# GiulioRomualdi/paper_romualdi_2022_icra_centroidal-mpc-walking

Hardware: AMD Instinct MI355X
Metric: centroidal-MPC solves/sec (batch, horizon=20) (higher is better)
Workload: dtype f32

## Files before the change

include/cmpc.h:

```cpp
#ifndef CMPC_H
#define CMPC_H

#include <stddef.h>

#ifdef __cplusplus
extern "C" {
#endif

typedef struct cmpc_handle_s* cmpc_handle;

typedef enum {
    CMPC_OK = 0,
    CMPC_ERR_ARG = -1,
    CMPC_ERR_HIP = -2,
    CMPC_ERR_NOT_CONVERGED = -3
} cmpc_status;

typedef struct {
    int horizon;
    double sampling_time;
    double friction_coefficient;
    double gravity;
    double com_weight[3];
    double angular_momentum_weight;
// ... 18 lines not shown
#define CMPC_FACTORS_HBM 2

#define CMPC_INFO 8

void cmpc_default_config(cmpc_config* cfg);
int cmpc_dims(int horizon, int* n_x, int* n_p, int* n_g, int* nnz_jac, int* nnz_hess);

double cmpc_default_tolerance(int horizon);
int cmpc_create(const cmpc_config* cfg, int batch, int device, cmpc_handle* out);
int cmpc_destroy(cmpc_handle h);
const char* cmpc_last_error(cmpc_handle h);
int cmpc_batch(cmpc_handle h);
void* cmpc_stream(cmpc_handle h);

int cmpc_solve_device(cmpc_handle h, const float* dP, const float* dX0, float* dX, float* dInfo,
                      void* stream);
int cmpc_solve_device_warm(cmpc_handle h, const float* dP, const float* dX0, float* dX, float* dInfo,
                           void* stream);
int cmpc_set_warm_policy(cmpc_handle h, int warm_budget, int restart_in_kernel);
int cmpc_solve(cmpc_handle h, const float* P, const float* X0, float* X, float* info);
float cmpc_last_solve_ms(cmpc_handle h);
int cmpc_set_timing(cmpc_handle h, int enabled);
int cmpc_test_poison_lds(cmpc_handle h);

typedef struct {
    double friction_coefficient;
    double com_weight[3];
    double angular_momentum_weight;
    double contact_position_weight;
    double force_rate_of_change_weight[3];
    double contact_force_symmetry_weight;
    double corners[2][4][3];
} cmpc_model;
#define CMPC_MODEL_DOUBLES 34
void cmpc_model_from_config(const cmpc_config* cfg, cmpc_model* model);
int cmpc_check_models(const cmpc_model* models, int batch);
int cmpc_set_models(cmpc_handle h, const cmpc_model* models);
int cmpc_set_models_device(cmpc_handle h, const cmpc_model* dModels, int* dOk, void* stream);

int cmpc_eval_nlp_device(cmpc_handle h, const float* dX, const float* dP, const float* dLamG,
                         float lam_f, float* dF, float* dG, float* dGradF, float* dJac,
                         float* dHess, void* stream);
int cmpc_nlp_sparsity(int horizon, int* jac_row, int* jac_col, int* hess_row, int* hess_col);
int cmpc_eval_nlp_grad_device(cmpc_handle h, const float* dX, const float* dP, const float* dLamG, float lam_f,
                              float* dGradX, float* dGradP, void* stream);

// ... 197 lines not shown
```

paper_romualdi_2022_icra_centroidal-mpc-walking_amd/_capi.py:

```python
from __future__ import annotations

import ctypes as C
import os

_HERE = os.path.dirname(os.path.abspath(__file__))
LIB_PATH = os.path.join(_HERE, os.environ.get("CMPC_LIB", "libcmpc_hip.so"))

INFO = 8
CERT = 8
SENS = 8


class CmpcConfig(C.Structure):
    _fields_ = [
        ("horizon", C.c_int),
        ("sampling_time", C.c_double),
        ("friction_coefficient", C.c_double),
        ("gravity", C.c_double),
        ("com_weight", C.c_double * 3),
        ("angular_momentum_weight", C.c_double),
        ("contact_position_weight", C.c_double),
        ("force_rate_of_change_weight", C.c_double * 3),
        ("contact_force_symmetry_weight", C.c_double),
        ("corners", C.c_double * 24),
# ... 52 lines not shown
class CmpcModel(C.Structure):
    _fields_ = [
        ("friction_coefficient", C.c_double),
        ("com_weight", C.c_double * 3),
        ("angular_momentum_weight", C.c_double),
        ("contact_position_weight", C.c_double),
        ("force_rate_of_change_weight", C.c_double * 3),
        ("contact_force_symmetry_weight", C.c_double),
        ("corners", C.c_double * 24),
    ]


MODEL_DOUBLES = 34


FACTORS = {None: 0, "auto": 0, "lds": 1, "hbm": 2}


EXPORTS = [
    "cmpc_default_config", "cmpc_dims", "cmpc_create", "cmpc_destroy", "cmpc_last_error",
    "cmpc_batch", "cmpc_stream", "cmpc_solve_device", "cmpc_solve", "cmpc_last_solve_ms", "cmpc_set_timing",
    "cmpc_eval_nlp_device", "cmpc_nlp_sparsity", "cmpc_set_state", "cmpc_set_reference",
    "cmpc_set_contacts", "cmpc_set_initial_guess", "cmpc_advance", "cmpc_get_solution",
    "cmpc_get_output", "cmpc_set_reference_from_planner", "cmpc_plant_step_device", "cmpc_test_poison_lds",
    "cmpc_compact_output_device", "cmpc_contacts_merge", "cmpc_contacts_merge_device", "cmpc_contacts_sample",
    "cmpc_contacts_sample_device", "cmpc_set_contact_lists", "cmpc_contacts_adjust", "cmpc_contacts_adjust_device",
    "cmpc_write_state_device", "cmpc_shift_solution_device", "cmpc_eval_nlp_grad_device", "cmpc_solve_device_warm", "cmpc_set_warm_policy",
    "cmpc_get_parameters", "cmpc_get_parameters_device", "cmpc_allgather_compact_device",
    "cmpc_rollout_tick_device", "cmpc_write_reference_from_planner_device", "cmpc_default_tolerance",
    "cmpc_contacts_force_sample_time", "cmpc_contacts_force_sample_time_device",
    "cmpc_model_from_config", "cmpc_check_models", "cmpc_set_models", "cmpc_set_models_device",
    "cmpc_set_multiplier_output", "cmpc_get_multipliers_device", "cmpc_get_multipliers", "cmpc_kkt_certificate_device",
    "cmpc_value_gradient_device", "cmpc_solution_jvp_device", "cmpc_solution_vjp_device",
    "cmpc_sensitivity_workspace_bytes", "cmpc_solution_jvp_model_device", "cmpc_solution_vjp_model_device", "cmpc_model_value_gradient_device",
    "cmpc_plant_step_jvp_device", "cmpc_plant_step_vjp_device", "cmpc_contacts_position_vjp_device", "cmpc_rollout_tick_vjp_device",
    "cmpc_solution_jvp_rot_device", "cmpc_solution_vjp_rot_device", "cmpc_rotation_value_gradient_device", "cmpc_contacts_rotation_vjp_device",
    "cmpc_plant_step_jvp_rot_device", "cmpc_plant_step_vjp_rot_device", "cmpc_contacts_orientation_vjp_device", "cmpc_rollout_tick_vjp_rot_device",
    "cmpc_plant_step_jvp_cols_device", "cmpc_contacts_jvp_device", "cmpc_rollout_tick_jvp_device",
    "cmpc_rollout_record", "cmpc_rollout_record_device", "cmpc_rollout_outcome_init_device", "cmpc_cold_start_device", "cmpc_rollout_walk_device",
]

_lib = None


def lib():
    global _lib
    if _lib is None:
# ... 114 lines not shown
```

paper_romualdi_2022_icra_centroidal-mpc-walking_amd/csrc/cmpc_api.hip:

```cpp
#include "../../include/cmpc.h"
#include "cmpc_contacts.h"
#include "cmpc_device.h"

#include <algorithm>
#include <cmath>
#include <cstdio>
#include <cstdlib>
#include <cstring>
#include <dlfcn.h>
#include <string>
#include <vector>

extern "C" size_t cmpc_solver_lds_bytes(int N, int factors_global);
extern "C" int cmpc_launch_solver(const CmpcParams* prm, size_t lds_bytes, hipStream_t stream);
extern "C" int cmpc_prepare_solver(int N, int factors_global, size_t lds_bytes);
extern "C" int cmpc_launch_nlp_eval(const CmpcParams* prm, const float* dX, const float* dP, const float* dLamG,
                                    float lam_f, float* dF, float* dG, float* dGradF, float* dJac, float* dHess,
                                    hipStream_t stream);
extern "C" int cmpc_launch_nlp_grad(const CmpcParams* prm, const float* dX, const float* dP, const float* dLamG, float lam_f, float* dGradX,
                                    float* dGradP, hipStream_t stream);
extern "C" int cmpc_launch_multipliers(const CmpcParams* prm, const float* dX, const float* dP, float* dLamG, hipStream_t stream);
extern "C" int cmpc_launch_kkt_certificate(const CmpcParams* prm, const float* dX, const float* dP, const float* dLamG, float* dCert, hipStream_t stream);
extern "C" int cmpc_launch_value_gradient(const CmpcParams* prm, const float* dX, const float* dP, const float* dLamG, float* dGradP, hipStream_t stream);
extern "C" int cmpc_launch_sensitivity(const CmpcConsts* kc, int kc_per_problem, int N, int b0, int nb, const float* dX, const float* dP, const float* dLamG,
// ... 673 lines not shown
    int rc = cmpc_launch_nlp_grad(&p, dX, dP, dLamG, lam_f, dGradX, dGradP, stream ? (hipStream_t)stream : h->stream);
    if (rc != 0) return fail(h, CMPC_ERR_HIP, std::string("nlp grad launch: ") + hipGetErrorString((hipError_t)rc));
    return CMPC_OK;
}

int cmpc_set_multiplier_output(cmpc_handle h, int enabled)
{
    if (!h) return fail(h, CMPC_ERR_ARG, "cmpc_set_multiplier_output: null handle");
    HIPCHK(h, hipSetDevice(h->device));
    if (enabled && !h->dDuals) {
        const size_t nd = (size_t)h->B * (CMPC_NS * (h->cfg.horizon + 1) + 2 * CMPC_NI * h->cfg.horizon);
        HIPCHK(h, hipMalloc(&h->dDuals, sizeof(float) * nd));
        HIPCHK(h, hipMemsetAsync(h->dDuals, 0, sizeof(float) * nd, h->stream));
        HIPCHK(h, hipStreamSynchronize(h->stream));
    } else if (!enabled && h->dDuals && !h->warm_duals) {
        HIPCHK(h, hipDeviceSynchronize());
        HIPCHK(h, hipFree(h->dDuals));
        h->dDuals = nullptr;
    }
    h->mult_out = enabled != 0;
    return CMPC_OK;
}

int cmpc_get_multipliers_device(cmpc_handle h, const float* dX, const float* dP, float* dLamG, void* stream)
{
    if (!h || !dX || !dP || !dLamG) return fail(h, CMPC_ERR_ARG, "cmpc_get_multipliers_device: null argument");
    if (!h->mult_out || !h->dDuals) return fail(h, CMPC_ERR_ARG, "cmpc_get_multipliers_device: the multiplier output is off (cmpc_set_multiplier_output)");
    HIPCHK(h, hipSetDevice(h->device));
    CmpcParams p;
    fill_params(h, p);
    int rc = cmpc_launch_multipliers(&p, dX, dP, dLamG, stream ? (hipStream_t)stream : h->stream);
    if (rc != 0) return fail(h, CMPC_ERR_HIP, std::string("multipliers launch: ") + hipGetErrorString((hipError_t)rc));
    return CMPC_OK;
}

int cmpc_get_multipliers(cmpc_handle h, float* LamG)
{
    if (!h || !LamG) return fail(h, CMPC_ERR_ARG, "cmpc_get_multipliers: null argument");
    if (!h->have_solution) return fail(h, CMPC_ERR_ARG, "cmpc_get_multipliers: no solution yet (cmpc_advance)");
    HIPCHK(h, hipSetDevice(h->device));
    const size_t n = (size_t)h->B * h->L.ng;
    if (!h->dLamG) HIPCHK(h, hipMalloc(&h->dLamG, sizeof(float) * n));
    int rc = cmpc_get_multipliers_device(h, h->dX, h->dP, h->dLamG, nullptr);
    if (rc != CMPC_OK) return rc;
    HIPCHK(h, hipMemcpyAsync(LamG, h->dLamG, sizeof(float) * n, hipMemcpyDeviceToHost, h->stream));
    HIPCHK(h, hipStreamSynchronize(h->stream));
// ... 1027 lines not shown
```

paper_romualdi_2022_icra_centroidal-mpc-walking_amd/csrc/cmpc_solver.hip:

```cpp
#include "cmpc_device.h"

#include <cstdlib>
#include <type_traits>
#include <map>
#include <mutex>

#define NS CMPC_NS
#define NF CMPC_NF
#define NQ CMPC_NQ
#define NU CMPC_NU
#define NXA CMPC_NXA
#define NI CMPC_NI
#define PLD 39
#define GLD 30
#define RLD 36
#define NPAN 46
#define GEO 36
#define SQ_TILE_WAVES 6
#define SQ_SPIN_MAX (1 << 20)
#define SQ_PUB_FLOATS (10 * NPAN * 4 + 128 * 4)
#define ZLD 36
#define MSET (NU * RLD + NPAN * RLD + NS * 16)
#define NTRI 256
#define ID_STRIP_LEN 68
#define ID_STRIPS (4 * ID_STRIP_LEN)
#define DSET_F (3 * NU + 3 * NS + 3 + 108)
#define DSET_I (3 * NU + 3 * NS + 3)
#define REC_UB 0
#define REC_WT 576
#define REC_ZERO 572
#define REC_N CMPC_REC_N
constexpr int SWEEP_UNROLL = 4;
constexpr int DELTA_UNROLL = 4;

namespace {

#ifdef CMPC_PROFILE
__device__ long long g_prof[128];
__device__ float g_trace[64 * 8];
#define PROF_DECL long long pt_ = __builtin_amdgcn_s_memtime()
#define PROF(slot) do { long long n_ = __builtin_amdgcn_s_memtime(); if (threadIdx.x == 0 && blockIdx.x == 0) g_prof[slot] += n_ - pt_; pt_ = n_; } while (0)
#define PROF2_DECL long long pt2_ = __builtin_amdgcn_s_memtime()
#define PROF3(slot) do { long long n_ = __builtin_amdgcn_s_memtime(); if (threadIdx.x == 192 && blockIdx.x == 0) g_prof[slot] += n_ - pt2_; pt2_ = n_; } while (0)
#define PROF4(slot) do { long long n_ = __builtin_amdgcn_s_memtime(); if (threadIdx.x == 128 && blockIdx.x == 0) g_prof[slot] += n_ - pt2_; pt2_ = n_; } while (0)
#define PROF2(slot) do { long long n_ = __builtin_amdgcn_s_memtime(); if (threadIdx.x == 0 && blockIdx.x == 0) g_prof[slot] += n_ - pt2_; pt2_ = n_; } while (0)
#define PROF5(slot) do { long long n_ = __builtin_amdgcn_s_memtime(); if (threadIdx.x == 216 && blockIdx.x == 0) g_prof[slot] += n_ - pt2_; pt2_ = n_; } while (0)
#define CPROF(i) do { if (ln == 0 && blockIdx.x == 0 && k < N) atomicAdd(reinterpret_cast<unsigned long long*>(&g_prof[32 + 5 * wv + (i)]), (unsigned long long)(__builtin_amdgcn_s_memtime() - pc0_)); } while (0)
#define CPROF2(i) do { if (ln == 0 && blockIdx.x == 0 && k < N) atomicAdd(reinterpret_cast<unsigned long long*>(&g_prof[64 + 8 * wv + (i)]), (unsigned long long)(__builtin_amdgcn_s_memtime() - pc0_)); } while (0)
#ifdef CMPC_PROFILE_LIGHT
#undef PROF2_DECL
#undef PROF2
#undef PROF3
#undef PROF4
#undef PROF5
#undef CPROF
#undef CPROF2
#define CPROF2(i)
#define PROF2_DECL
#define PROF2(slot)
#define PROF3(slot)
#define PROF4(slot)
#define PROF5(slot)
#define CPROF(i)
#define SQPROF_DECL
#define SQPROF(slot)
#else
#define SQPROF_DECL PROF_DECL
#define SQPROF(slot) PROF(slot)
#endif
#else
#define SQPROF_DECL
#define SQPROF(slot)
#define CPROF(i)
#define CPROF2(i)
#define PROF_DECL
#define PROF(slot)
#define PROF2_DECL
#define PROF2(slot)
#define PROF3(slot)
#define PROF4(slot)
#define PROF5(slot)
#endif

struct Ctx {
    CmpcIdx L;
    int N;
    const float* sp;
    float *S, *U, *T, *Z;
    float* LAM;
    float *dS, *dU, *dT, *dZ, *d;
    float *Lf;
    float *geoA;
    float *P0, *Qb, *G, *QuuF, *Pan, *Bval, *Aval, *arow, *ybuf, *fpv, *fpn;
    float *idstrip;
    float *ZT;
    double *QuuD1, *qs1;
    int *Brow, *Arow, *qmask;
    unsigned short* tri;
    double *QuuD, *pv, *pn, *qs, *Pd, *sig, *gco, *redd;
// ... 133 lines not shown
{
    const auto r = __builtin_amdgcn_permlane32_swap(__float_as_uint(v), __float_as_uint(v), false, false);
    return __uint_as_float(r[0]) + __uint_as_float(r[1]);
}
__device__ inline float oct_sum(float v)
{
    v += __uint_as_float(__builtin_amdgcn_update_dpp(0u, __float_as_uint(v), 0xB1, 0xF, 0xF, true));
    v += __uint_as_float(__builtin_amdgcn_update_dpp(0u, __float_as_uint(v), 0x4E, 0xF, 0xF, true));
    v += __uint_as_float(__builtin_amdgcn_update_dpp(0u, __float_as_uint(v), 0x141, 0xF, 0xF, true));
    return v;
}
__device__ inline float dot4(const float4& a, const float4& b) { return a.x * b.x + a.y * b.y + a.z * b.z + a.w * b.w; }

__device__ inline float gam_of(const Ctx& c, int ct, int k) { return c.sp[c.L.pGam(ct) + k]; }
__device__ inline float Rm(const float* R, int r, int cc) { return R[3 * cc + r]; }

__device__ inline bool qfree_compute(const Ctx& c, int k, int m)
{
    const int ct = m / 3, i = m % 3;
    const float lo = c.sp[c.L.pLo(ct) + 3 * k + i], hi = c.sp[c.L.pUp(ct) + 3 * k + i];
    return gam_of(c, ct, k) < 0.5f && (hi - lo) > 1e-9f;
}
__device__ inline bool qfree(const Ctx& c, int k, int m) { return (c.qmask[k] >> m) & 1; }
__device__ inline bool outside_subset(const Ctx& c, int ct, int k)
{
    const float g = gam_of(c, ct, k);
    if (g == 0.f) return false;
    if (g != 1.f) return true;
    int kp = -1;
    for (int j = k - 1; j >= 0 && kp < 0; --j) if (gam_of(c, ct, j) < 0.5f) kp = j;
    const float* R = c.sp + c.L.pR(ct) + 9 * k;
    const float* nom = c.sp + c.L.pNom(ct) + 3 * (k + 1);
    const float* lo = c.sp + c.L.pLo(ct) + 3 * k;
    const float* up = c.sp + c.L.pUp(ct) + 3 * k;
    if (kp < 0) {
        const float* cur = c.sp + c.L.pCur(ct);
        bool out = false;
        for (int i = 0; i < 3; ++i) {
            float v = 0.f;
            for (int a = 0; a < 3; ++a) v += Rm(R, a, i) * (cur[a] - nom[a]);
            out = out || !(v >= lo[i] - 1e-6f && v <= up[i] + 1e-6f);
        }
        return out;
    }
    const float* Rp = c.sp + c.L.pR(ct) + 9 * kp;
    const float* nomp = c.sp + c.L.pNom(ct) + 3 * (kp + 1);
    const float* lop = c.sp + c.L.pLo(ct) + 3 * kp;
    const float* upp = c.sp + c.L.pUp(ct) + 3 * kp;
    bool diff = false;
    for (int a = 0; a < 9; ++a) diff = diff || __float_as_int(R[a]) != __float_as_int(Rp[a]);
    for (int i = 0; i < 3; ++i)
        diff = diff || __float_as_int(nom[i]) != __float_as_int(nomp[i]) || __float_as_int(lo[i]) != __float_as_int(lop[i])
               || __float_as_int(up[i]) != __float_as_int(upp[i]);
    return diff;
}
__device__ inline float qlo(const Ctx& c, int k, int m) { return c.sp[c.L.pLo(m / 3) + 3 * k + m % 3]; }
__device__ inline float qhi(const Ctx& c, int k, int m) { return c.sp[c.L.pUp(m / 3) + 3 * k + m % 3]; }

__device__ inline void fric_row(const Ctx& c, const CmpcConsts& prm, int k, int i, float& a0, float& a1, float& a2)
{
    const int ct = i >> 4, face = i & 3;
    const float* R = c.sp + c.L.pR(ct) + 9 * k;
    const float sx = (face == 0 || face == 3) ? 1.f : -1.f;
    const float sy = (face < 2) ? 1.f : -1.f;
    const float nmu = -prm.mu_fr;
    a0 = __builtin_fmaf(nmu, Rm(R, 0, 2), __builtin_fmaf(sy, Rm(R, 0, 1), sx * Rm(R, 0, 0)));
    a1 = __builtin_fmaf(nmu, Rm(R, 1, 2), __builtin_fmaf(sy, Rm(R, 1, 1), sx * Rm(R, 1, 0)));
    a2 = __builtin_fmaf(nmu, Rm(R, 2, 2), __builtin_fmaf(sy, Rm(R, 2, 1), sx * Rm(R, 2, 0)));
}

__device__ inline bool row_active(const Ctx& c, int k, int i) { return i < 32 ? true : qfree(c, k, (i - 32) % 6); }

__device__ inline float row_val(const Ctx& c, const CmpcConsts& prm, int k, int i, const float* u)
{
    if (i < 32) {
        float a0, a1, a2;
// ... 2066 lines not shown
{
    CMPC_PHASE_PROLOGUE;
    const bool affine = __builtin_amdgcn_readfirstlane((int)affine_in) != 0;
    riccati_forward<NT, NC == 0 ? 1 : (FG ? 2 : SWEEP_UNROLL), FG, PART>(c, prm, tid, affine, 0);
}
template <int NT, int NC, bool FG>
__device__ __forceinline__ void phase_forward_sweep(lds_t lds, int Nrt, float* fg_base, bool affine_in)
{
    if (threadIdx.x < 64) phase_forward_part<NT, NC, FG, 1>(lds, Nrt, fg_base, affine_in);
}
template <int NT, int NC, bool FG>
__device__ __attribute__((noinline)) void phase_forward_tail(lds_t lds, int Nrt, float* fg_base, bool affine_in, int k0_in)
{
    CMPC_PHASE_PROLOGUE;
    const bool affine = __builtin_amdgcn_readfirstlane((int)affine_in) != 0;
    const int k0 = __builtin_amdgcn_readfirstlane(k0_in);
    riccati_forward<NT, 1, FG>(c, prm, tid, affine, k0);
}
template <int NT, int NC, bool FG>
__device__ __attribute__((noinline)) void phase_delta_part(lds_t lds, int Nrt, float* fg_base)
{
    CMPC_PHASE_PROLOGUE;
    riccati_delta<NC == 0 ? 1 : (FG ? 2 : DELTA_UNROLL), FG>(c, prm, tid);
}
template <int NT, int NC, bool FG>
__device__ __forceinline__ void phase_delta(lds_t lds, int Nrt, float* fg_base)
{
    if (threadIdx.x < 64) phase_delta_part<NT, NC, FG>(lds, Nrt, fg_base);
    __syncthreads();
}
template <int NT, int NC, bool FG>
__device__ __attribute__((noinline)) void phase_costate(lds_t lds, int Nrt, float* fg_base, float ap, bool exact_in)
{
    CMPC_PHASE_PROLOGUE;
    const bool use_exact = __builtin_amdgcn_readfirstlane((int)exact_in) != 0;
    costate_update(c, prm, tid, ap, use_exact);
}
__device__ inline float dual_extrapolate(float z, float dz) { return fmaxf(z + dz, 0.f); }

template <int NT, int NC, bool FG>
__device__ __attribute__((noinline)) void tail_polish(lds_t lds, int Nrt, float* fg_base, int k0_in, bool duals_in)
{
    CMPC_PHASE_PROLOGUE;
    const int k0 = __builtin_amdgcn_readfirstlane(k0_in);
    const bool duals = __builtin_amdgcn_readfirstlane((int)duals_in) != 0;
    bool last = false, blocked = true;
    for (int pi = 0; pi <= prm.tail_iters + 6 && !last; ++pi) {
        last = pi >= prm.tail_iters + 6 || (pi >= prm.tail_iters && !blocked);
        all_geo<NT>(c, prm, tid);
        for (int e = tid + NS * k0; e < NS * N; e += NT) c.d[e] = (float)defect(c, prm, e / NS, e % NS);
        __syncthreads();
// ... 150 lines not shown
        if (e % NU < NF) {
            l_fm = fmaxf(l_fm, fabsf(c.U[e]));
            if (e >= NU * kt) l_tail = fmaxf(l_tail, fabsf(du));
        }
    }
    float m3[3] = {l_all, l_tail, l_fm};
    block_maxn<NT, 3>(m3, c.red, tid);
    if (!(m3[0] < INFINITY)) return false;
    const int k0 = (prm.tail_stages > 0 && m3[1] > prm.tail_trigger * m3[2]) ? kt : N;
    if (k0 < N) step_lengths<NT>(c, tid, 0.999f, ap, ad, 0, k0);
    for (int e = tid; e < NS * (k0 < N ? k0 + 1 : N + 1); e += NT) c.S[e] += ap * c.dS[e];
    for (int e = tid; e < NU * k0; e += NT) c.U[e] += ap * c.dU[e];
    if (duals)
        for (int e = tid; e < NI * k0; e += NT) {
            const float tn = c.T[e] + ap * c.dT[e], zn = dual_extrapolate(c.Z[e], c.dZ[e]);
            if (fabsf(tn) < INFINITY && fabsf(zn) < INFINITY) { c.T[e] = tn; c.Z[e] = zn; }
        }
    __syncthreads();
    if (k0 == N) return false;
    tail_polish<NT, NC, FG>(lds, N, fg_base, k0, duals);
    return true;
}

template <int NT, int NC, bool FG>
__device__ __attribute__((noinline)) int phase_setup(lds_t lds, int Nrt, float* fg_base, const float* gp)
{
    CMPC_PHASE_PROLOGUE;
    float* spw = const_cast<float*>(c.sp);
    for (int e = tid; e < NTRI; e += NT) {
        int i = (int)((sqrtf(8.f * (float)e + 1.f) - 1.f) * 0.5f);
        while ((i + 1) * (i + 2) / 2 <= e) ++i;
        while (i * (i + 1) / 2 > e) --i;
        c.tri[e] = (unsigned short)((i << 8) | (e - i * (i + 1) / 2));
    }
    for (int e = tid; e < ID_STRIPS; e += NT) c.idstrip[e] = (e % ID_STRIP_LEN) == 32 + e / ID_STRIP_LEN ? 1.f : 0.f;
    for (int e = tid; e < c.L.np(); e += NT) spw[e] = gp[e];
    if (tid == 0) c.flag[0] = 0;
    __syncthreads();
    if (tid < N) {
        int m = 0;
#pragma unroll
        for (int q = 0; q < NQ; ++q) m |= qfree_compute(c, tid, q) ? (1 << q) : 0;
        c.qmask[tid] = m;
    }
    if (tid < 2 * N && outside_subset(c, tid / N, tid % N)) c.flag[0] = 1;
    __syncthreads();
    return __builtin_amdgcn_readfirstlane(c.flag[0]);
}

template <int NT, int NC, bool FG>
__device__ __attribute__((noinline)) int phase_init(lds_t lds, int Nrt, float* fg_base, const float* x0, const float* dprev, int flags, float mu_init,
                                                    float t_floor)
{
    CMPC_PHASE_PROLOGUE;
    const bool cold = (flags & 1) != 0, use_duals = (flags & 2) != 0, use_mult = (flags & 4) != 0;
    for (int e = tid; e < NS * (N + 1); e += NT) {
        const int k = e / NS, i = e % NS;
        float v;
        if (k == 0) {
            if (i < 9) v = c.sp[c.L.pCom0() + i];
            else v = c.sp[c.L.pCur((i - 9) / 3) + (i - 9) % 3];
        } else if (cold) v = i < 3 ? c.sp[c.L.pCom0() + i] : (i < 9 ? 0.f : c.sp[c.L.pNom((i - 9) / 3) + 3 * k + (i - 9) % 3]);
        else if (i < 9) v = x0[c.L.oCom() + 3 * (N + 1) * (i / 3) + 3 * k + i % 3];
        else v = x0[c.L.oPos((i - 9) / 3) + 3 * k + (i - 9) % 3];
        c.S[e] = v;
        c.LAM[e] = (use_duals && !cold) ? dprev[NS * (k < N ? k + 1 : N) + i] : 0.f;
    }
    for (int e = tid; e < NU * N; e += NT) {
        const int k = e / NU, m = e % NU;
        float v = 0.f;
        if (m < NF) v = cold ? (m % 3 == 2 ? 0.125f * prm.grav : 0.f) : x0[c.L.oF(m / 12, (m % 12) / 3) + 3 * k + m % 3];
        else {
            const int q = m - 24, ct = q / 3, i = q % 3;
            if (qfree(c, k, q)) {
                const float* R = c.sp + c.L.pR(ct) + 9 * k;
                const float lo = qlo(c, k, q), hi = qhi(c, k, q), push = 0.01f * (hi - lo);
                for (int a = 0; a < 3 && !cold; ++a)
                    v += Rm(R, a, i) * (x0[c.L.oPos(ct) + 3 * (k + 1) + a] - c.sp[c.L.pNom(ct) + 3 * (k + 1) + a]);
                v = fminf(fmaxf(v, lo + push), hi - push);
            } else if (gam_of(c, ct, k) < 0.5f) v = qlo(c, k, q);
        }
        c.U[e] = v;
    }
    __syncthreads();
    for (int e = tid; e < NI * N; e += NT) {
        const int k = e / NI, i = e % NI;
        float t = 1.f, z = 0.f;
        if (row_active(c, k, i)) {
            t = -row_val(c, prm, k, i, c.U + NU * k);
            if (i < 32) t = fmaxf(t, t_floor);
            z = mu_init / t;
            if (use_mult && !cold) {
                const int kk = k + 1 < N ? k + 1 : N - 1;
                z = fmaxf(z, dprev[NS * (N + 1) + NI * N + NI * kk + i]);
            }
        }
        c.T[e] = t; c.Z[e] = z;
    }
    __syncthreads();
    int nrow = 0;
    for (int k = 0; k < N; ++k)
        for (int i = 32; i < NI; ++i) nrow += row_active(c, k, i) ? 1 : 0;
    return __builtin_amdgcn_readfirstlane(nrow + 32 * N);
}

template <int NT, int NC, bool FG>
__device__ __attribute__((noinline)) float phase_multipliers(lds_t lds, int Nrt, float* fg_base, int mode_in, float a_in, int nrow_in)
{
    CMPC_PHASE_PROLOGUE;
    const int mode = __builtin_amdgcn_readfirstlane(mode_in), nrow = __builtin_amdgcn_readfirstlane(nrow_in);
    const float a = uniform_f(a_in);
    float out = a;
    if (mode == 0) {
        for (int e = tid; e < NI * N; e += NT) c.Z[e] *= a;
    } else if (mode == 1) {
        double l2 = 0.0;
        for (int e = tid; e < NI * N; e += NT)
            if (row_active(c, e / NI, e % NI)) {
                const float t = c.T[e];
                float z = c.Z[e];
                if (t * z > 10.f * a) { z = 10.f * a / t; c.Z[e] = z; }
                l2 += (double)t * z;
            }
        out = (float)(block_sum<NT>(l2, c.redd, tid) / (double)nrow);
    } else {
        for (int e = tid; e < NI * N; e += NT) c.dZ[e] = row_active(c, e / NI, e % NI) ? a : 0.f;
// ... 200 lines not shown
            for (int e = tid; e < NS * N; e += NT) c.d[e] = 0.f;
            __syncthreads();
            if (tid < 64) costate_scan<true>(c, prm, tid, 0.f, false, c.LAM);
            __syncthreads();
        }
        for (int e = tid; e < NS * (N + 1); e += NT) dq[e] = e < NS ? (e == 0 ? (float)status : 0.f) : c.LAM[e];
        for (int e = tid; e < NI * N; e += NT) { dq[NS * (N + 1) + e] = c.T[e]; dq[NS * (N + 1) + NI * N + e] = c.Z[e]; }
    }
#ifdef CMPC_PROFILE
    if (prm.hwid_probe) {
        __syncthreads();
        if ((threadIdx.x & 63) == 0) x[threadIdx.x >> 6] = (float)(__builtin_amdgcn_s_getreg((31 << 11) | 4) & 0xffff);
    }
#endif
}

template <int NT, int NC, bool FG>
__global__ __launch_bounds__(NT, FG ? 3 : 1) void cmpc_solve_kernel(CmpcParams kp)
{
    extern __shared__ __attribute__((aligned(16))) char smem[];
    const int b = blockIdx.x;
    const int tid = threadIdx.x;
    const int N = NC > 0 ? NC : kp.N;
    {
        int* z = reinterpret_cast<int*>(smem);
        for (int e = tid; e < kp.lds_words; e += NT) z[e] = 0;
    }
    __syncthreads();
    {
        const int* src = reinterpret_cast<const int*>(kp.kc_per_problem ? kp.kc + b : kp.kc);
        int* dst = reinterpret_cast<int*>(smem);
        for (int e = tid; e < (int)(sizeof(CmpcConsts) / 4); e += NT) dst[e] = src[e];
    }
    const CmpcConsts& prm = *reinterpret_cast<const CmpcConsts*>(smem);
    const long long t_start = __builtin_amdgcn_s_memtime();
    unsigned ldsv = (unsigned)(unsigned long long)(lds_t)smem;
    asm volatile("" : "+s"(ldsv));
    const lds_t lds = (lds_t)(unsigned long long)ldsv;
    float* const fg_base = FG ? kp.scratch + (size_t)b * kp.scratch_stride : nullptr;
    const CmpcIdx L{N};
    __syncthreads();
    const bool outside = (phase_setup<NT, NC, FG>(lds, N, fg_base, kp.P + (size_t)b * L.np()) != 0) | (prm.model_bad != 0);
    int status = 1, sg = 0, it_total = 0;
    float err = 0.f, ep = 0.f, mu_cur = 0.f, step_out = 0.f, step_prev = 0.f;
    float* const dq = kp.duals ? kp.duals + (size_t)b * (NS * (N + 1) + 2 * NI * N) : nullptr;
    if (outside) {
        phase_init<NT, NC, FG>(lds, N, fg_base, kp.X0 + (size_t)b * L.nx(), dq, 0, kp.mu_init, kp.t_floor);
        status = 3;
    }
    for (int pass = 0; pass < 2 && !outside; ++pass) {
        const float mu_init = pass ? 0.1f : kp.mu_init, t_floor = pass ? 1e-2f : kp.t_floor, mu_adapt = pass ? 3.5f : kp.mu_adapt;
        step_out = step_prev = 0.f;
        const bool use_duals = kp.warm && kp.warm_duals && kp.duals;
        const int nrow = phase_init<NT, NC, FG>(lds, N, fg_base, kp.X0 + (size_t)b * L.nx(), dq,
                                                (pass > 0 ? 1 : 0) | (use_duals ? 2 : 0) | (use_duals && kp.warm_duals > 1 ? 4 : 0), mu_init, t_floor);
        int it = 0;
        status = 1;
        bool finishing = false;
        const int budget = (kp.warm && pass == 0 && kp.warm_budget > 0 && kp.warm_budget < prm.max_iter) ? kp.warm_budget : prm.max_iter;
        for (it = 0; it < budget + 1; ++it) {
            if (it == budget && !finishing) break;
            PROF_DECL;
            const Resid rs = phase_residuals<NT, NC, FG>(lds, N, fg_base, nrow);
            ep = rs.ep;
            const float ec = rs.ec;
            mu_cur = rs.mu;
            if (!(ep < INFINITY)) { status = 2; err = INFINITY; break; }
            if (it == 0 && mu_adapt > 0.f) {
                const float mu0 = fminf(fmaxf(mu_adapt * ep * ep, 0.03f), 0.5f);
                phase_multipliers<NT, NC, FG>(lds, N, fg_base, 0, mu0 / mu_cur, nrow);
                mu_cur = mu0;
            }
            if (kp.warm && pass == 0 && it > 0 && ec > 100.f * mu_cur && ec > 0.1f) {
                mu_cur = phase_multipliers<NT, NC, FG>(lds, N, fg_base, 1, mu_cur, nrow);
                sg += 100;
            }
            PROF(10);
            float est = step_out;
// ... 13 lines not shown
            int fail = 1;
            bool resync = false;
            for (int attempt = 0; attempt < 4; ++attempt) {
                fail = phase_backward<NT, NC, FG>(lds, N, fg_base, exact, reg, centring ? prm.mu_min : 0.f);
                if (!fail) break;
                __syncthreads();
                if (fail & 2) {
                    sg += 1000000;
                    if (!resync) { resync = true; --attempt; continue; }
                }
                ++sg; exact = false;
                if (attempt > 0) reg *= 1e3f;
            }
            if (fail) { if (!finishing) status = 2; break; }
            PROF(11);
            float sigma = 0.f, mu_t = prm.mu_min;
            if (centring) {
                phase_multipliers<NT, NC, FG>(lds, N, fg_base, 2, prm.mu_min, nrow);
            } else {
                phase_forward_sweep<NT, NC, FG>(lds, N, fg_base, true);
                PROF(12);
                if (finishing) {
                    phase_forward_part<NT, NC, FG, 2>(lds, N, fg_base, true);
                    if (phase_finish<NT, NC, FG>(lds, N, fg_base, dq != nullptr)) sg += 100000;
                    ++it;
                    break;
                }
                Centre ce;
                if constexpr (NC > 0) ce = phase_affine_post<NT, NC, FG>(lds, N, fg_base, mu_cur, nrow);
                else {
                    phase_forward_part<NT, NC, FG, 2>(lds, N, fg_base, true);
                    const StepLen sa = phase_step_lengths<NT, NC, FG>(lds, N, fg_base, 1.f);
                    ce = phase_corrector_targets<NT, NC, FG>(lds, N, fg_base, sa.ap, sa.ad, mu_cur, nrow);
                }
                sigma = ce.sigma; mu_t = ce.mu_t;
                PROF(13);
                phase_delta<NT, NC, FG>(lds, N, fg_base);
                PROF(14);
            }
            phase_forward_sweep<NT, NC, FG>(lds, N, fg_base, false);
            PROF(15);
            float ap, ad, step;
            if constexpr (NC > 0) {
                const FinalStep fs = phase_final_post<NT, NC, FG>(lds, N, fg_base, fmaxf(0.99f, 1.f - mu_t), exact);
                ap = fs.ap; ad = fs.ad; step = fs.step;
                PROF(16);
            } else {
// ... 5 lines not shown
                step = phase_update<NT, NC, FG>(lds, N, fg_base, ap, ad);
            }
            step_prev = step_out;
            step_out = step;
            err = fmaxf(ep, ec);
    #ifdef CMPC_PROFILE
            if (tid == 0 && b == 0 && it < 64) {
                float* tr = g_trace + 8 * it;
                tr[0] = mu_cur; tr[1] = ep; tr[2] = ec; tr[3] = step; tr[4] = ap; tr[5] = ad; tr[6] = sigma; tr[7] = mu_t;
            }
    #endif
            PROF(17);
            if (err <= prm.tol && step <= prm.step_tol) {
                status = 0;
                if (!prm.final_extrap) { ++it; break; }
                finishing = true;
            }
        }
        it_total += it;
        if (status == 0 || !kp.warm || pass > 0 || kp.warm_no_restart) break;
        sg += 10000;
        __syncthreads();
    }
    phase_export<NT, NC, FG>(lds, N, fg_base, kp.X + (size_t)b * L.nx(), dq, status);
    if (kp.info && tid == 0) {
        float* inf = kp.info + (size_t)b * CMPC_INFO_N;
        inf[0] = (float)it_total; inf[1] = err; inf[2] = mu_cur; inf[3] = (float)sg; inf[4] = ep; inf[5] = (float)status;
        inf[6] = (float)(__builtin_amdgcn_s_memtime() - t_start); inf[7] = step_out;
    }
}

}

extern "C" size_t cmpc_solver_lds_bytes(int N, int factors_global)
{
    CmpcLayout L;
    cmpc_layout_init(L, N);
    const size_t dbl = 90 + 40 + 40 + 16 + 40 + 4 * NI + 8 + (factors_global ? 0 : 90 + 16);
    const size_t work = factors_global ? ((NXA * PLD + 3) & ~3) + NS * 16 + ((NXA * GLD + 3) & ~3) : (size_t)MSET + NS * 16 + SQ_PUB_FLOATS + 128;
    const size_t flt = (size_t)NU * RLD + (size_t)NPAN * RLD + 96 + ID_STRIPS + ((L.np + 3) & ~3)
                       + ((size_t)NS * (N + 1) + (size_t)NU * N + ((factors_global && N > CMPC_TZ_LDS_NMAX) ? 0 : 2 * (size_t)NI * N)) + (size_t)NS * N + (size_t)NS * (N + 1)
                       + (size_t)GEO * N + work + 2 * DSET_F + 40 + 40 + 24
                       + 2 * DSET_I + 4 + CMPC_NMAX + NTRI / 2 + (factors_global ? 0 : (size_t)REC_N * N);
    return ((sizeof(CmpcConsts) + 15) & ~(size_t)15) + dbl * 8 + flt * 4;
}

#ifdef CMPC_PROFILE
extern "C" int cmpc_profile_read(long long* out, int reset)
{
    hipError_t e = hipMemcpyFromSymbol(out, HIP_SYMBOL(g_prof), sizeof(long long) * 128);
    if (reset) { long long z[128] = {0}; (void)hipMemcpyToSymbol(HIP_SYMBOL(g_prof), z, sizeof(z)); }
    return (int)e;
}
extern "C" int cmpc_trace_read(float* out) { return (int)hipMemcpyFromSymbol(out, HIP_SYMBOL(g_trace), sizeof(float) * 64 * 8); }
#endif

typedef void (*cmpc_kernel_t)(CmpcParams);
static cmpc_kernel_t solver_variant(int N, bool factors_global, int& nthreads)
{
    constexpr int NT = 256, NR = 512;
    if (factors_global) {
        nthreads = NT;
        return N == 20 ? cmpc_solve_kernel<NT, 20, true> : (N == 30 ? cmpc_solve_kernel<NT, 30, true> : cmpc_solve_kernel<NT, 0, true>);
    }
    nthreads = NR;
    switch (N) {
        case 10: return cmpc_solve_kernel<NR, 10, false>;
        case 12: return cmpc_solve_kernel<NR, 12, false>;
        case 13: return cmpc_solve_kernel<NR, 13, false>;
        case 15: return cmpc_solve_kernel<NR, 15, false>;
        case 20: return cmpc_solve_kernel<NR, 20, false>;
        case 22: return cmpc_solve_kernel<NR, 22, false>;
        default: return cmpc_solve_kernel<NR, 0, false>;
    }
// ... 27 lines not shown
```

Measured before the change: 370,200.

## Prefetch setup inputs into registers, precompute tri table, streamline solver init

Moves the global loads of per-problem constants, parameters and a compile-time triangular index table into registers before the LDS zeroing, so their latency overlaps the clear. Replaces per-thread sqrt-based tri index computation with a constant table. Also stages the warm-start x0 in LDS, precomputes the previous swing stage with a bitmask instead of a backward scan, counts active rows with ballot/popcount, and uses non-short-circuit boolean ops. It also adds per-workgroup profiling macros (compiled out by default) and a test hook for warm duals. The costs are higher register pressure from the prefetch arrays and extra LDS reuse of the dS buffer.

```diff
diff --git a/include/cmpc.h b/include/cmpc.h
--- a/include/cmpc.h
+++ b/include/cmpc.h
@@ -64,6 +64,7 @@
 float cmpc_last_solve_ms(cmpc_handle h);
 int cmpc_set_timing(cmpc_handle h, int enabled);
 int cmpc_test_poison_lds(cmpc_handle h);
+int cmpc_test_set_warm_duals(cmpc_handle h, int mode);
 
 typedef struct {
     double friction_coefficient;
diff --git a/paper_romualdi_2022_icra_centroidal-mpc-walking_amd/_capi.py b/paper_romualdi_2022_icra_centroidal-mpc-walking_amd/_capi.py
--- a/paper_romualdi_2022_icra_centroidal-mpc-walking_amd/_capi.py
+++ b/paper_romualdi_2022_icra_centroidal-mpc-walking_amd/_capi.py
@@ -98,7 +98,7 @@
     "cmpc_batch", "cmpc_stream", "cmpc_solve_device", "cmpc_solve", "cmpc_last_solve_ms", "cmpc_set_timing",
     "cmpc_eval_nlp_device", "cmpc_nlp_sparsity", "cmpc_set_state", "cmpc_set_reference",
     "cmpc_set_contacts", "cmpc_set_initial_guess", "cmpc_advance", "cmpc_get_solution",
-    "cmpc_get_output", "cmpc_set_reference_from_planner", "cmpc_plant_step_device", "cmpc_test_poison_lds",
+    "cmpc_get_output", "cmpc_set_reference_from_planner", "cmpc_plant_step_device", "cmpc_test_poison_lds", "cmpc_test_set_warm_duals",
     "cmpc_compact_output_device", "cmpc_contacts_merge", "cmpc_contacts_merge_device", "cmpc_contacts_sample",
     "cmpc_contacts_sample_device", "cmpc_set_contact_lists", "cmpc_contacts_adjust", "cmpc_contacts_adjust_device",
     "cmpc_write_state_device", "cmpc_shift_solution_device", "cmpc_eval_nlp_grad_device", "cmpc_solve_device_warm", "cmpc_set_warm_policy",
diff --git a/paper_romualdi_2022_icra_centroidal-mpc-walking_amd/csrc/cmpc_api.hip b/paper_romualdi_2022_icra_centroidal-mpc-walking_amd/csrc/cmpc_api.hip
--- a/paper_romualdi_2022_icra_centroidal-mpc-walking_amd/csrc/cmpc_api.hip
+++ b/paper_romualdi_2022_icra_centroidal-mpc-walking_amd/csrc/cmpc_api.hip
@@ -719,6 +719,20 @@
     return CMPC_OK;
 }
 
+int cmpc_test_set_warm_duals(cmpc_handle h, int mode)
+{
+    if (!h || mode < 0 || mode > 2) return fail(h, CMPC_ERR_ARG, "cmpc_test_set_warm_duals: null handle or mode outside 0..2");
+    HIPCHK(h, hipSetDevice(h->device));
+    if (mode && !h->dDuals) {
+        const size_t nd = (size_t)h->B * (CMPC_NS * (h->cfg.horizon + 1) + 2 * CMPC_NI * h->cfg.horizon);
+        HIPCHK(h, hipMalloc(&h->dDuals, sizeof(float) * nd));
+        HIPCHK(h, hipMemsetAsync(h->dDuals, 0, sizeof(float) * nd, h->stream));
+        HIPCHK(h, hipStreamSynchronize(h->stream));
+    }
+    h->warm_duals = mode;
+    return CMPC_OK;
+}
+
 int cmpc_get_multipliers_device(cmpc_handle h, const float* dX, const float* dP, float* dLamG, void* stream)
 {
     if (!h || !dX || !dP || !dLamG) return fail(h, CMPC_ERR_ARG, "cmpc_get_multipliers_device: null argument");
diff --git a/paper_romualdi_2022_icra_centroidal-mpc-walking_amd/csrc/cmpc_solver.hip b/paper_romualdi_2022_icra_centroidal-mpc-walking_amd/csrc/cmpc_solver.hip
--- a/paper_romualdi_2022_icra_centroidal-mpc-walking_amd/csrc/cmpc_solver.hip
+++ b/paper_romualdi_2022_icra_centroidal-mpc-walking_amd/csrc/cmpc_solver.hip
@@ -40,6 +40,14 @@
 __device__ float g_trace[64 * 8];
 #define PROF_DECL long long pt_ = __builtin_amdgcn_s_memtime()
 #define PROF(slot) do { long long n_ = __builtin_amdgcn_s_memtime(); if (threadIdx.x == 0 && blockIdx.x == 0) g_prof[slot] += n_ - pt_; pt_ = n_; } while (0)
+constexpr int PROF_WG = 1024;
+__device__ long long g_prof_wg[PROF_WG * 8];
+#define LPROF_DECL long long lp_ = __builtin_amdgcn_s_memtime(); const long long lp0_ = lp_
+#define LPROF_MARK() do { lp_ = __builtin_amdgcn_s_memtime(); } while (0)
+#define LPROF(slot) do { long long n_ = __builtin_amdgcn_s_memtime(); if (threadIdx.x == 0 && blockIdx.x < PROF_WG) g_prof_wg[8 * blockIdx.x + (slot)] += n_ - lp_; lp_ = n_; } while (0)
+#define LPROF_TOTAL(slot) do { if (threadIdx.x == 0 && blockIdx.x < PROF_WG) g_prof_wg[8 * blockIdx.x + (slot)] += __builtin_amdgcn_s_memtime() - lp0_; } while (0)
+#define LPROF_LEAVE() do { if (threadIdx.x == 0 && blockIdx.x < PROF_WG) g_prof_wg[8 * blockIdx.x + 7] = __builtin_amdgcn_s_memtime(); } while (0)
+#define LPROF_BACK(slot) do { if (threadIdx.x == 0 && blockIdx.x < PROF_WG) g_prof_wg[8 * blockIdx.x + (slot)] += __builtin_amdgcn_s_memtime() - g_prof_wg[8 * blockIdx.x + 7]; } while (0)
 #define PROF2_DECL long long pt2_ = __builtin_amdgcn_s_memtime()
 #define PROF3(slot) do { long long n_ = __builtin_amdgcn_s_memtime(); if (threadIdx.x == 192 && blockIdx.x == 0) g_prof[slot] += n_ - pt2_; pt2_ = n_; } while (0)
 #define PROF4(slot) do { long long n_ = __builtin_amdgcn_s_memtime(); if (threadIdx.x == 128 && blockIdx.x == 0) g_prof[slot] += n_ - pt2_; pt2_ = n_; } while (0)
@@ -75,6 +83,12 @@
 #define CPROF2(i)
 #define PROF_DECL
 #define PROF(slot)
+#define LPROF_DECL
+#define LPROF_MARK()
+#define LPROF(slot)
+#define LPROF_TOTAL(slot)
+#define LPROF_LEAVE()
+#define LPROF_BACK(slot)
 #define PROF2_DECL
 #define PROF2(slot)
 #define PROF3(slot)
@@ -254,13 +268,11 @@
     return gam_of(c, ct, k) < 0.5f && (hi - lo) > 1e-9f;
 }
 __device__ inline bool qfree(const Ctx& c, int k, int m) { return (c.qmask[k] >> m) & 1; }
-__device__ inline bool outside_subset(const Ctx& c, int ct, int k)
+__device__ inline bool outside_subset(const Ctx& c, int ct, int k, int kp)
 {
     const float g = gam_of(c, ct, k);
     if (g == 0.f) return false;
     if (g != 1.f) return true;
-    int kp = -1;
-    for (int j = k - 1; j >= 0 && kp < 0; --j) if (gam_of(c, ct, j) < 0.5f) kp = j;
     const float* R = c.sp + c.L.pR(ct) + 9 * k;
     const float* nom = c.sp + c.L.pNom(ct) + 3 * (k + 1);
     const float* lo = c.sp + c.L.pLo(ct) + 3 * k;
@@ -271,7 +283,7 @@
         for (int i = 0; i < 3; ++i) {
             float v = 0.f;
             for (int a = 0; a < 3; ++a) v += Rm(R, a, i) * (cur[a] - nom[a]);
-            out = out || !(v >= lo[i] - 1e-6f && v <= up[i] + 1e-6f);
+            out = out | !((v >= lo[i] - 1e-6f) & (v <= up[i] + 1e-6f));
         }
         return out;
     }
@@ -280,10 +292,10 @@
     const float* lop = c.sp + c.L.pLo(ct) + 3 * kp;
     const float* upp = c.sp + c.L.pUp(ct) + 3 * kp;
     bool diff = false;
-    for (int a = 0; a < 9; ++a) diff = diff || __float_as_int(R[a]) != __float_as_int(Rp[a]);
+    for (int a = 0; a < 9; ++a) diff = diff | (__float_as_int(R[a]) != __float_as_int(Rp[a]));
     for (int i = 0; i < 3; ++i)
-        diff = diff || __float_as_int(nom[i]) != __float_as_int(nomp[i]) || __float_as_int(lo[i]) != __float_as_int(lop[i])
-               || __float_as_int(up[i]) != __float_as_int(upp[i]);
+        diff = diff | (__float_as_int(nom[i]) != __float_as_int(nomp[i])) | (__float_as_int(lo[i]) != __float_as_int(lop[i]))
+               | (__float_as_int(up[i]) != __float_as_int(upp[i]));
     return diff;
 }
 __device__ inline float qlo(const Ctx& c, int k, int m) { return c.sp[c.L.pLo(m / 3) + 3 * k + m % 3]; }
@@ -2396,11 +2408,15 @@
 {
     CMPC_PHASE_PROLOGUE;
     riccati_delta<NC == 0 ? 1 : (FG ? 2 : DELTA_UNROLL), FG>(c, prm, tid);
+    LPROF_LEAVE();
 }
 template <int NT, int NC, bool FG>
 __device__ __forceinline__ void phase_delta(lds_t lds, int Nrt, float* fg_base)
 {
-    if (threadIdx.x < 64) phase_delta_part<NT, NC, FG>(lds, Nrt, fg_base);
+    if (threadIdx.x < 64) {
+        phase_delta_part<NT, NC, FG>(lds, Nrt, fg_base);
+        LPROF_BACK(5);
+    }
     __syncthreads();
 }
 template <int NT, int NC, bool FG>
@@ -2597,19 +2613,23 @@
     return true;
 }
 
+struct alignas(16) TriTable { unsigned short v[NTRI]; };
+constexpr TriTable make_tri_table()
+{
+    TriTable t{};
+    int e = 0;
+    for (int i = 0; e < NTRI; ++i)
+        for (int j = 0; j <= i && e < NTRI; ++j) t.v[e++] = (unsigned short)((i << 8) | j);
+    return t;
+}
+__constant__ const TriTable TRI_TABLE = make_tri_table();
 template <int NT, int NC, bool FG>
-__device__ __attribute__((noinline)) int phase_setup(lds_t lds, int Nrt, float* fg_base, const float* gp)
+__device__ __attribute__((noinline)) int phase_setup(lds_t lds, int Nrt, float* fg_base)
 {
     CMPC_PHASE_PROLOGUE;
-    float* spw = const_cast<float*>(c.sp);
-    for (int e = tid; e < NTRI; e += NT) {
-        int i = (int)((sqrtf(8.f * (float)e + 1.f) - 1.f) * 0.5f);
-        while ((i + 1) * (i + 2) / 2 <= e) ++i;
-        while (i * (i + 1) / 2 > e) --i;
-        c.tri[e] = (unsigned short)((i << 8) | (e - i * (i + 1) / 2));
-    }
-    for (int e = tid; e < ID_STRIPS; e += NT) c.idstrip[e] = (e % ID_STRIP_LEN) == 32 + e / ID_STRIP_LEN ? 1.f : 0.f;
-    for (int e = tid; e < c.L.np(); e += NT) spw[e] = gp[e];
+    static_assert(ID_STRIPS == 4 * ID_STRIP_LEN, "four strips");
+    for (int e = tid; e < ID_STRIPS; e += NT)
+        c.idstrip[e] = ((e == 32) | (e == ID_STRIP_LEN + 33) | (e == 2 * ID_STRIP_LEN + 34) | (e == 3 * ID_STRIP_LEN + 35)) ? 1.f : 0.f;
     if (tid == 0) c.flag[0] = 0;
     __syncthreads();
     if (tid < N) {
@@ -2618,7 +2638,14 @@
         for (int q = 0; q < NQ; ++q) m |= qfree_compute(c, tid, q) ? (1 << q) : 0;
         c.qmask[tid] = m;
     }
-    if (tid < 2 * N && outside_subset(c, tid / N, tid % N)) c.flag[0] = 1;
+    if (tid < 2 * N) {
+        static_assert(CMPC_NMAX <= 64, "one bit per stage");
+        const int ct = tid / N, k = tid % N;
+        unsigned long long swing = 0;
+        for (int j = 0; j < N; ++j) swing |= (unsigned long long)(gam_of(c, ct, j) < 0.5f ? 1 : 0) << j;
+        const unsigned long long before = swing & ((1ull << k) - 1ull);
+        if (outside_subset(c, ct, k, before ? 63 - __clzll((long long)before) : -1)) c.flag[0] = 1;
+    }
     __syncthreads();
     return __builtin_amdgcn_readfirstlane(c.flag[0]);
 }
@@ -2628,7 +2655,24 @@
                                                     float t_floor)
 {
     CMPC_PHASE_PROLOGUE;
+    flags = __builtin_amdgcn_readfirstlane(flags);
     const bool cold = (flags & 1) != 0, use_duals = (flags & 2) != 0, use_mult = (flags & 4) != 0;
+    typedef const __attribute__((address_space(1))) float* gfloat_t;
+    const gfloat_t gx = (gfloat_t)x0, gd = (gfloat_t)dprev;
+    float* const xs = c.dS;
+    const bool from_x0 = !cold, lam_prev = use_duals && !cold, z_prev = use_mult && !cold;
+    if (from_x0)
+        for (int e = tid; e < c.L.nx(); e += NT) xs[e] = gx[e];
+    for (int e = tid; e < NS * (N + 1); e += NT) {
+        const int k = e / NS, i = e % NS;
+        c.LAM[e] = lam_prev ? gd[NS * (k < N ? k + 1 : N) + i] : 0.f;
+    }
+    if (z_prev)
+        for (int e = tid; e < NI * N; e += NT) {
+            const int k = e / NI, i = e % NI, kk = k + 1 < N ? k + 1 : N - 1;
+            c.Z[e] = gd[NS * (N + 1) + NI * N + NI * kk + i];
+        }
+    if (from_x0) __syncthreads();
     for (int e = tid; e < NS * (N + 1); e += NT) {
         const int k = e / NS, i = e % NS;
         float v;
@@ -2636,28 +2680,29 @@
             if (i < 9) v = c.sp[c.L.pCom0() + i];
             else v = c.sp[c.L.pCur((i - 9) / 3) + (i - 9) % 3];
         } else if (cold) v = i < 3 ? c.sp[c.L.pCom0() + i] : (i < 9 ? 0.f : c.sp[c.L.pNom((i - 9) / 3) + 3 * k + (i - 9) % 3]);
-        else if (i < 9) v = x0[c.L.oCom() + 3 * (N + 1) * (i / 3) + 3 * k + i % 3];
-        else v = x0[c.L.oPos((i - 9) / 3) + 3 * k + (i - 9) % 3];
+        else if (i < 9) v = xs[c.L.oCom() + 3 * (N + 1) * (i / 3) + 3 * k + i % 3];
+        else v = xs[c.L.oPos((i - 9) / 3) + 3 * k + (i - 9) % 3];
         c.S[e] = v;
-        c.LAM[e] = (use_duals && !cold) ? dprev[NS * (k < N ? k + 1 : N) + i] : 0.f;
     }
     for (int e = tid; e < NU * N; e += NT) {
         const int k = e / NU, m = e % NU;
         float v = 0.f;
-        if (m < NF) v = cold ? (m % 3 == 2 ? 0.125f * prm.grav : 0.f) : x0[c.L.oF(m / 12, (m % 12) / 3) + 3 * k + m % 3];
+        if (m < NF) v = cold ? (m % 3 == 2 ? 0.125f * prm.grav : 0.f) : xs[c.L.oF(m / 12, (m % 12) / 3) + 3 * k + m % 3];
         else {
             const int q = m - 24, ct = q / 3, i = q % 3;
             if (qfree(c, k, q)) {
                 const float* R = c.sp + c.L.pR(ct) + 9 * k;
                 const float lo = qlo(c, k, q), hi = qhi(c, k, q), push = 0.01f * (hi - lo);
                 for (int a = 0; a < 3 && !cold; ++a)
-                    v += Rm(R, a, i) * (x0[c.L.oPos(ct) + 3 * (k + 1) + a] - c.sp[c.L.pNom(ct) + 3 * (k + 1) + a]);
+                    v += Rm(R, a, i) * (xs[c.L.oPos(ct) + 3 * (k + 1) + a] - c.sp[c.L.pNom(ct) + 3 * (k + 1) + a]);
                 v = fminf(fmaxf(v, lo + push), hi - push);
             } else if (gam_of(c, ct, k) < 0.5f) v = qlo(c, k, q);
         }
         c.U[e] = v;
     }
     __syncthreads();
+    if (from_x0)
+        for (int e = tid; e < c.L.nx(); e += NT) xs[e] = 0.f;
     for (int e = tid; e < NI * N; e += NT) {
         const int k = e / NI, i = e % NI;
         float t = 1.f, z = 0.f;
@@ -2665,18 +2710,20 @@
             t = -row_val(c, prm, k, i, c.U + NU * k);
             if (i < 32) t = fmaxf(t, t_floor);
             z = mu_init / t;
-            if (use_mult && !cold) {
-                const int kk = k + 1 < N ? k + 1 : N - 1;
-                z = fmaxf(z, dprev[NS * (N + 1) + NI * N + NI * kk + i]);
-            }
+            if (z_prev) z = fmaxf(z, c.Z[e]);
         }
         c.T[e] = t; c.Z[e] = z;
     }
     __syncthreads();
-    int nrow = 0;
-    for (int k = 0; k < N; ++k)
-        for (int i = 32; i < NI; ++i) nrow += row_active(c, k, i) ? 1 : 0;
-    return __builtin_amdgcn_readfirstlane(nrow + 32 * N);
+    static_assert((NI - 32) % NQ == 0, "row_active maps row i >= 32 to component (i - 32) % NQ");
+    int nfree = 0;
+    for (int k0 = 0; k0 < N; k0 += 64) {
+        const int k = k0 + (tid & 63);
+        const int m = k < N ? c.qmask[k] : 0;
+#pragma unroll
+        for (int q = 0; q < NQ; ++q) nfree += __popcll(__ballot((m >> q) & 1));
+    }
+    return __builtin_amdgcn_readfirstlane((NI - 32) / NQ * nfree + 32 * N);
 }
 
 template <int NT, int NC, bool FG>
@@ -2923,15 +2970,41 @@
     const int b = blockIdx.x;
     const int tid = threadIdx.x;
     const int N = NC > 0 ? NC : kp.N;
+    LPROF_DECL;
+    constexpr int KW = (int)(sizeof(CmpcConsts) / 4), KT = (KW + NT - 1) / NT;
+    constexpr int PT = (50 * (NC > 0 ? NC : CMPC_NMAX) + 27 + NT - 1) / NT;
+    constexpr int TT = (NTRI / 2 + NT - 1) / NT;
+    const CmpcIdx L{N};
+    int kreg[KT], treg[TT];
+    float preg[PT];
+    {
+        const int* src = reinterpret_cast<const int*>(kp.kc_per_problem ? kp.kc + b : kp.kc);
+        const float* gp = kp.P + (size_t)b * L.np();
+        const int* tsrc = reinterpret_cast<const int*>(TRI_TABLE.v);
+#pragma unroll
+        for (int j = 0; j < KT; ++j) { const int e = tid + j * NT; kreg[j] = e < KW ? src[e] : 0; }
+#pragma unroll
+        for (int j = 0; j < PT; ++j) { const int e = tid + j * NT; preg[j] = e < L.np() ? gp[e] : 0.f; }
+#pragma unroll
+        for (int j = 0; j < TT; ++j) { const int e = tid + j * NT; treg[j] = e < NTRI / 2 ? tsrc[e] : 0; }
+    }
     {
         int* z = reinterpret_cast<int*>(smem);
         for (int e = tid; e < kp.lds_words; e += NT) z[e] = 0;
     }
     __syncthreads();
     {
-        const int* src = reinterpret_cast<const int*>(kp.kc_per_problem ? kp.kc + b : kp.kc);
         int* dst = reinterpret_cast<int*>(smem);
-        for (int e = tid; e < (int)(sizeof(CmpcConsts) / 4); e += NT) dst[e] = src[e];
+#pragma unroll
+        for (int j = 0; j < KT; ++j) { const int e = tid + j * NT; if (e < KW) dst[e] = kreg[j]; }
+        Ctx c;
+        make_ctx<FG>(c, smem, N, nullptr);
+        float* spw = const_cast<float*>(c.sp);
+        int* tw = reinterpret_cast<int*>(c.tri);
+#pragma unroll
+        for (int j = 0; j < PT; ++j) { const int e = tid + j * NT; if (e < L.np()) spw[e] = preg[j]; }
+#pragma unroll
+        for (int j = 0; j < TT; ++j) { const int e = tid + j * NT; if (e < NTRI / 2) tw[e] = treg[j]; }
     }
     const CmpcConsts& prm = *reinterpret_cast<const CmpcConsts*>(smem);
     const long long t_start = __builtin_amdgcn_s_memtime();
@@ -2939,22 +3012,26 @@
     asm volatile("" : "+s"(ldsv));
     const lds_t lds = (lds_t)(unsigned long long)ldsv;
     float* const fg_base = FG ? kp.scratch + (size_t)b * kp.scratch_stride : nullptr;
-    const CmpcIdx L{N};
     __syncthreads();
-    const bool outside = (phase_setup<NT, NC, FG>(lds, N, fg_base, kp.P + (size_t)b * L.np()) != 0) | (prm.model_bad != 0);
+    LPROF(0);
+    const bool outside = (phase_setup<NT, NC, FG>(lds, N, fg_base) != 0) | (prm.model_bad != 0);
+    LPROF(1);
     int status = 1, sg = 0, it_total = 0;
     float err = 0.f, ep = 0.f, mu_cur = 0.f, step_out = 0.f, step_prev = 0.f;
     float* const dq = kp.duals ? kp.duals + (size_t)b * (NS * (N + 1) + 2 * NI * N) : nullptr;
     if (outside) {
         phase_init<NT, NC, FG>(lds, N, fg_base, kp.X0 + (size_t)b * L.nx(), dq, 0, kp.mu_init, kp.t_floor);
+        LPROF(2);
         status = 3;
     }
     for (int pass = 0; pass < 2 && !outside; ++pass) {
         const float mu_init = pass ? 0.1f : kp.mu_init, t_floor = pass ? 1e-2f : kp.t_floor, mu_adapt = pass ? 3.5f : kp.mu_adapt;
         step_out = step_prev = 0.f;
         const bool use_duals = kp.warm && kp.warm_duals && kp.duals;
+        LPROF_MARK();
         const int nrow = phase_init<NT, NC, FG>(lds, N, fg_base, kp.X0 + (size_t)b * L.nx(), dq,
                                                 (pass > 0 ? 1 : 0) | (use_duals ? 2 : 0) | (use_duals && kp.warm_duals > 1 ? 4 : 0), mu_init, t_floor);
+        LPROF(2);
         int it = 0;
         status = 1;
         bool finishing = false;
@@ -3014,7 +3091,9 @@
                 PROF(12);
                 if (finishing) {
                     phase_forward_part<NT, NC, FG, 2>(lds, N, fg_base, true);
+                    LPROF_MARK();
                     if (phase_finish<NT, NC, FG>(lds, N, fg_base, dq != nullptr)) sg += 100000;
+                    LPROF(3);
                     ++it;
                     break;
                 }
@@ -3066,7 +3145,10 @@
         sg += 10000;
         __syncthreads();
     }
+    LPROF_MARK();
     phase_export<NT, NC, FG>(lds, N, fg_base, kp.X + (size_t)b * L.nx(), dq, status);
+    LPROF(4);
+    LPROF_TOTAL(6);
     if (kp.info && tid == 0) {
         float* inf = kp.info + (size_t)b * CMPC_INFO_N;
         inf[0] = (float)it_total; inf[1] = err; inf[2] = mu_cur; inf[3] = (float)sg; inf[4] = ep; inf[5] = (float)status;
@@ -3094,6 +3176,16 @@
 {
     hipError_t e = hipMemcpyFromSymbol(out, HIP_SYMBOL(g_prof), sizeof(long long) * 128);
     if (reset) { long long z[128] = {0}; (void)hipMemcpyToSymbol(HIP_SYMBOL(g_prof), z, sizeof(z)); }
+    return (int)e;
+}
+extern "C" int cmpc_profile_wg_read(long long* out, int nwg, int reset)
+{
+    if (nwg < 0 || nwg > PROF_WG) return (int)hipErrorInvalidValue;
+    hipError_t e = hipMemcpyFromSymbol(out, HIP_SYMBOL(g_prof_wg), sizeof(long long) * 8 * nwg);
+    if (reset) {
+        static long long z[PROF_WG * 8];
+        (void)hipMemcpyToSymbol(HIP_SYMBOL(g_prof_wg), z, sizeof(z));
+    }
     return (int)e;
 }
 extern "C" int cmpc_trace_read(float* out) { return (int)hipMemcpyFromSymbol(out, HIP_SYMBOL(g_trace), sizeof(float) * 64 * 8); }
```

New measurement: 370,900 (median of 5 runs). Within noise of the previous version (+0.2%).
